# iden3/snarkjs

Hardware: NVIDIA H100
Metric: groth16_proofs_per_sec (higher is better)
Workload: dtype u32x8 (256-bit modular integers, 32-bit limbs)

## Files before the change

### snarkjs_b200/csrc/msm.cuh

```cuda
#pragma once
#include <cuda_runtime.h>
#include "ec.cuh"
#include "msm_geom.h"

namespace sb {

static constexpr int MSM_SEG = 32;
static constexpr int MSM_ACC_THREADS = 128;
static constexpr int MSM_RED_CHUNK = 16;
static constexpr uint32_t MSM_INVALID_KEY = 0xffffffffu;
static constexpr int MSM_COUNTS_SEG = 8;

extern int g_msm_force_c;

__host__ inline MsmGeom msm_choose(uint64_t n, uint32_t scalar_bytes, int fr_bits, bool precomp) {
    int eff = (int)(8 * scalar_bytes) < fr_bits ? (int)(8 * scalar_bytes) : fr_bits;
    int best_c = 3; double best = 1e300;
    for (int c = 3; c <= 22; c++) {
        int weff = (eff + 1 + c - 1) / c, top = eff + 1 - (weff - 1) * c;
        if (weff > 1 && top < c - 5) continue;
        double buckets = (precomp ? 1.0 : (double)weff) * (double)(1u << (c - 1));
        double cost = (double)weff * (double)n * 10.0 + buckets * 60.0;
        if (cost < best) { best = cost; best_c = c; }
    }
    if (g_msm_force_c) best_c = g_msm_force_c;
    MsmGeom g; g.c = best_c; g.W = (int)((8 * scalar_bytes + 1 + best_c - 1) / best_c); g.B = 1u << (best_c - 1);
    return g;
}
__host__ inline MsmGeom msm_geometry_precomp(uint64_t n_set, uint32_t scalar_bytes, int fr_bits = 254) {
    int l2 = 0; while ((1ull << (l2 + 1)) <= n_set) l2++;
    int cmax = l2; if (cmax > 22) cmax = 22; if (cmax < 8) cmax = 8;
    int c = 8;
    for (int cc = cmax; cc >= 8; cc--) {
        int weff = (fr_bits + 1 + cc - 1) / cc, top = fr_bits + 1 - (weff - 1) * cc;
        if (weff > 1 && top < cc - 5) continue;
        c = cc; break;
    }
    if (g_msm_force_c) c = g_msm_force_c;
    MsmGeom g; g.c = c; g.W = (int)((8 * scalar_bytes + 1 + c - 1) / c); g.B = 1u << (c - 1);
    g.precomp = 1; g.stride = n_set; g.first = 0;
    return g;
}
__host__ inline MsmGeom msm_geometry(uint64_t n, uint32_t scalar_bytes, int fr_bits = 254) {
    return msm_choose(n, scalar_bytes, fr_bits, false);
}

template <class F> __device__ __forceinline__ void load_affine(const Affine<F>* __restrict__ bases, uint32_t idx, F& x, F& y) {
    constexpr int NV = sizeof(F) / 16;
    const uint4* p = reinterpret_cast<const uint4*>(bases + idx);
    uint4* dx = reinterpret_cast<uint4*>(&x);
    uint4* dy = reinterpret_cast<uint4*>(&y);
#pragma unroll
    for (int k = 0; k < NV; k++) dx[k] = __ldg(p + k);
#pragma unroll
    for (int k = 0; k < NV; k++) dy[k] = __ldg(p + NV + k);
}
template <class T> __device__ __forceinline__ void store_vec(T* dst, const T& v) {
    constexpr int NV = sizeof(T) / 16;
    const uint4* s = reinterpret_cast<const uint4*>(&v);
    uint4* d = reinterpret_cast<uint4*>(dst);
#pragma unroll
    for (int k = 0; k < NV; k++) d[k] = s[k];
}
template <class T> __device__ __forceinline__ T load_vec(const T* src) {
    constexpr int NV = sizeof(T) / 16;
    T v; const uint4* s = reinterpret_cast<const uint4*>(src);
    uint4* d = reinterpret_cast<uint4*>(&v);
#pragma unroll
    for (int k = 0; k < NV; k++) d[k] = s[k];
    return v;
}

template <class P> __device__ __forceinline__ Fp<P> PairInvF(const Fp<P>& a) { return Fp<P>::inv_binary(a); }
template <class P> __device__ __forceinline__ Fp2<P> PairInvF(const Fp2<P>& a) { return Fp2<P>::inv(a); }

template <class F, int MINB>
__global__ void __launch_bounds__(MSM_ACC_THREADS, MINB)
k_accumulate(const Affine<F>* __restrict__ bases, const uint32_t* __restrict__ keys, const uint32_t* __restrict__ vals,
             const uint64_t* __restrict__ counts, XYZZ<F>* __restrict__ buckets,
             XYZZ<F>* __restrict__ heads, uint32_t* __restrict__ head_keys) {
    const uint64_t M = counts[0];
    const uint32_t seg = (uint32_t)counts[MSM_COUNTS_SEG];
    uint64_t t = blockIdx.x * (uint64_t)blockDim.x + threadIdx.x;
    uint64_t lo = t * seg;
    if (lo >= M) return;
    uint64_t hi = lo + seg < M ? lo + seg : M;
    const F one = F::one();
    XYZZ<F> acc = XYZZ<F>::inf();
    uint32_t cur = keys[lo];
    bool first = true;
    for (uint64_t e = lo; e < hi; e++) {
        uint32_t k = keys[e], v = vals ? vals[e] : (uint32_t)e;
        if (k != cur) {
            if (first) { store_vec(heads + t, acc); head_keys[t] = cur; first = false; }
            else store_vec(buckets + cur, acc);
            acc = XYZZ<F>::inf(); cur = k;
        }
        F px, py;
        load_affine<F>(bases, v & 0x7fffffffu, px, py);
        if (!(px.is_zero() & py.is_zero())) {
            py = F::cneg(py, (v >> 31) != 0);
            acc.add_affine(px, py, one);
        }
    }
    if (first) { store_vec(heads + t, acc); head_keys[t] = cur; }
    else store_vec(buckets + cur, acc);
}

static constexpr int MSM_SHORT_RUN = 8;
template <class F, int MINB>
__global__ void __launch_bounds__(MSM_ACC_THREADS, MINB)
k_fold_short(const XYZZ<F>* __restrict__ heads, const uint32_t* __restrict__ keys_in, uint32_t* __restrict__ keys_out,
             const uint64_t* __restrict__ counts, XYZZ<F>* __restrict__ buckets) {
    const uint64_t M = counts[1];
    uint64_t t = blockIdx.x * (uint64_t)blockDim.x + threadIdx.x;
    if (t >= M) return;
    const uint32_t k = keys_in[t];
    uint64_t start = t; int back = 0;
    while (start > 0 && back < MSM_SHORT_RUN && keys_in[start - 1] == k) { start--; back++; }
    bool is_short = back < MSM_SHORT_RUN;
    uint64_t len = 0;
    if (is_short) {
        len = 1;
        while (start + len < M && len <= (uint64_t)MSM_SHORT_RUN && keys_in[start + len] == k) len++;
        is_short = len <= (uint64_t)MSM_SHORT_RUN;
    }
    keys_out[t] = is_short ? MSM_INVALID_KEY : k;
    if (!is_short || start != t) return;
    XYZZ<F> acc = load_vec(buckets + k);
    for (uint64_t e = 0; e < len; e++) { XYZZ<F> p = load_vec(heads + t + e); acc.add_i(p); }
    store_vec(buckets + k, acc);
}

template <class F>
__global__ void __launch_bounds__(MSM_ACC_THREADS)
k_fold(const XYZZ<F>* __restrict__ in, const uint32_t* __restrict__ in_keys, const uint64_t* __restrict__ counts, int level,
       XYZZ<F>* __restrict__ buckets, XYZZ<F>* __restrict__ heads, uint32_t* __restrict__ head_keys) {
    const uint64_t M = counts[level];
    const bool last = M <= MSM_SEG;
    uint64_t t = blockIdx.x * (uint64_t)blockDim.x + threadIdx.x;
    uint64_t lo = t * MSM_SEG;
    if (lo >= M) return;
    uint64_t hi = lo + MSM_SEG < M ? lo + MSM_SEG : M;
    XYZZ<F> acc = XYZZ<F>::inf();
    uint32_t cur = in_keys[lo];
    bool first = !last;
    auto flush = [&]() __attribute__((always_inline)) {
        if (first) { store_vec(heads + t, acc); head_keys[t] = cur; first = false; }
        else if (cur != MSM_INVALID_KEY) { XYZZ<F> b = load_vec(buckets + cur); b.add_i(acc); store_vec(buckets + cur, b); }
    };
    for (uint64_t e = lo; e < hi; e++) {
        uint32_t k = in_keys[e];
        if (k != cur) { flush(); acc = XYZZ<F>::inf(); cur = k; }
        if (k != MSM_INVALID_KEY) { XYZZ<F> p = load_vec(in + e); acc.add_i(p); }
    }
    flush();
}

template <class F>
__global__ void __launch_bounds__(128)
k_reduce(const XYZZ<F>* __restrict__ buckets, MsmGeom g, XYZZ<F>* __restrict__ partials, uint32_t ctas_per_window) {
    extern __shared__ uint4 smem_raw[];
    XYZZ<F>* sm = reinterpret_cast<XYZZ<F>*>(smem_raw);
    const uint32_t w = blockIdx.x / ctas_per_window, cta = blockIdx.x % ctas_per_window;
    const uint32_t L = g.B < (uint32_t)MSM_RED_CHUNK ? g.B : MSM_RED_CHUNK;
    const uint32_t chunks = g.B / L;
    const uint32_t j = cta * blockDim.x + threadIdx.x;
    XYZZ<F> part = XYZZ<F>::inf();
    if (j < chunks) {
        const XYZZ<F>* bk = buckets + (uint64_t)w * g.B + (uint64_t)j * L;
        XYZZ<F> run = XYZZ<F>::inf(), sum = XYZZ<F>::inf();
        for (int b = (int)L - 1; b >= 0; b--) {
            XYZZ<F> p = load_vec(bk + b);
            run.add_i(p);
            sum.add_i(run);
        }
        uint32_t k = j * L;
        if (k) {
            int top = 31 - __clz(k);
            part = run;
            for (int bit = top - 1; bit >= 0; bit--) {
                part = XYZZ<F>::dbl(part);
                if ((k >> bit) & 1) part.add_i(run);
            }
        }
        part.add_i(sum);
    }
    store_vec(sm + threadIdx.x, part);
    __syncthreads();
    for (uint32_t s = blockDim.x >> 1; s > 0; s >>= 1) {
        if (threadIdx.x < s) {
            XYZZ<F> a = load_vec(sm + threadIdx.x), b = load_vec(sm + threadIdx.x + s);
            a.add_i(b);
            store_vec(sm + threadIdx.x, a);
        }
        __syncthreads();
    }
    if (threadIdx.x == 0) store_vec(partials + (uint64_t)w * ctas_per_window + cta, load_vec(sm));
}

template <class F>
__global__ void __launch_bounds__(32)
k_window_sum(const XYZZ<F>* __restrict__ partials, uint32_t per_window, XYZZ<F>* __restrict__ out) {
    extern __shared__ uint4 smem_raw[];
    XYZZ<F>* sm = reinterpret_cast<XYZZ<F>*>(smem_raw);
    XYZZ<F> acc = XYZZ<F>::inf();
    for (uint32_t i = threadIdx.x; i < per_window; i += 32) { XYZZ<F> p = load_vec(partials + (uint64_t)blockIdx.x * per_window + i); acc.add_i(p); }
    store_vec(sm + threadIdx.x, acc);
    __syncwarp();
    for (uint32_t s = 16; s > 0; s >>= 1) {
        if (threadIdx.x < s) { XYZZ<F> a = load_vec(sm + threadIdx.x), b = load_vec(sm + threadIdx.x + s); a.add_i(b); store_vec(sm + threadIdx.x, a); }
        __syncwarp();
    }
    if (threadIdx.x == 0) store_vec(out + blockIdx.x, load_vec(sm));
}


struct AxisJob { const void* in; void* out; uint64_t total; uint32_t S; uint32_t log_inner; };

template <class F, int MINB>
__global__ void __launch_bounds__(128, MINB)
k_axis_sum(AxisJob j0, AxisJob j1) {
    const AxisJob j = blockIdx.y ? j1 : j0;
    const uint64_t gid = blockIdx.x * (uint64_t)blockDim.x + threadIdx.x;
    if (gid >= j.total) return;
    const uint64_t o = gid >> j.log_inner, i = gid & ((1ull << j.log_inner) - 1);
    const XYZZ<F>* p = (const XYZZ<F>*)j.in + ((o * j.S) << j.log_inner) + i;
    XYZZ<F> acc = load_vec(p);
#pragma unroll 1
    for (uint32_t s = 1; s < j.S; s++) { XYZZ<F> v = load_vec(p + ((uint64_t)s << j.log_inner)); acc.add_i(v); }
    store_vec((XYZZ<F>*)j.out + gid, acc);
}

template <class F> __device__ __forceinline__ XYZZ<F> shfl_down_pt(const XYZZ<F>& v, int d) {
    constexpr int NW32 = sizeof(XYZZ<F>) / 4;
    union U { XYZZ<F> p; uint32_t w[NW32]; __device__ U() {} };
    U a, r; a.p = v;
#pragma unroll
    for (int k = 0; k < NW32; k++) r.w[k] = __shfl_down_sync(0xffffffffu, a.w[k], d);
    return r.p;
}
template <class F> __device__ __forceinline__ void warp_weighted_sum(XYZZ<F> v, XYZZ<F>& T, XYZZ<F>& W) {
    const int lane = threadIdx.x & 31;
#pragma unroll 1
    for (int d = 1; d < 32; d <<= 1) { XYZZ<F> o = shfl_down_pt<F>(v, d); if (lane + d < 32) v.add_i(o); }
    T = v;
    XYZZ<F> x = lane ? v : XYZZ<F>::inf();
#pragma unroll 1
    for (int d = 16; d >= 1; d >>= 1) { XYZZ<F> o = shfl_down_pt<F>(x, d); if (lane < d) x.add_i(o); }
    W = x;
}
template <class F> __device__ __forceinline__ XYZZ<F> warp_sum(XYZZ<F> x) {
    const int lane = threadIdx.x & 31;
#pragma unroll 1
    for (int d = 16; d >= 1; d >>= 1) { XYZZ<F> o = shfl_down_pt<F>(x, d); if (lane < d) x.add_i(o); }
    return x;
}

template <class F>
__global__ void __launch_bounds__(128)
k_ws_chunks(const XYZZ<F>* __restrict__ vecR, uint32_t lenR, const XYZZ<F>* __restrict__ vecC, uint32_t lenC, uint32_t NW, XYZZ<F>* __restrict__ tw) {
    const uint32_t nR = (lenR + 31) / 32, nC = (lenC + 31) / 32, per = nR + nC;
    const uint32_t wid = blockIdx.x * (blockDim.x >> 5) + (threadIdx.x >> 5), lane = threadIdx.x & 31;
    if (wid >= NW * per) return;
    const uint32_t w = wid / per, jj = wid % per;
    const bool isR = jj < nR;
    const uint32_t j = isR ? jj : jj - nR, len = isR ? lenR : lenC, idx = j * 32 + lane;
    const XYZZ<F>* vec = (isR ? vecR : vecC) + (uint64_t)w * len;
    XYZZ<F> v = XYZZ<F>::inf();
    if (idx < len) v = load_vec(vec + idx);
    XYZZ<F> T, W;
    warp_weighted_sum<F>(v, T, W);
    if (lane == 0) { store_vec(tw + 2 * (uint64_t)wid, T); store_vec(tw + 2 * (uint64_t)wid + 1, W); }
}

template <class F>
__global__ void __launch_bounds__(128)
k_ws_final(const XYZZ<F>* __restrict__ tw, uint32_t nR, uint32_t nC, XYZZ<F>* __restrict__ out) {
    const uint32_t warp = threadIdx.x >> 5, lane = threadIdx.x & 31, per = nR + nC;
    const XYZZ<F>* base = tw + 2 * (uint64_t)blockIdx.x * per;
    const bool r_side = warp < 2;
    const uint32_t cnt = r_side ? nR : nC, off = r_side ? 0 : nR;
    XYZZ<F> v = XYZZ<F>::inf();
    if (lane < cnt) v = load_vec(base + 2 * (uint64_t)(off + lane) + (warp & 1));
    XYZZ<F>* o = out + 5 * (uint64_t)blockIdx.x;
    if ((warp & 1) == 0) {
        XYZZ<F> tot, res;
        warp_weighted_sum<F>(v, tot, res);
        if (lane == 0) { store_vec(o + (r_side ? 0 : 2), res); if (!r_side) store_vec(o + 4, tot); }
    } else {
        XYZZ<F> res = warp_sum<F>(v);
        if (lane == 0) store_vec(o + (r_side ? 1 : 3), res);
    }
}

template <class F>
__global__ void __launch_bounds__(128)
k_axis_tree(AxisJob j0, AxisJob j1) {
    const AxisJob j = blockIdx.y ? j1 : j0;
    const uint64_t wid = blockIdx.x * (uint64_t)(blockDim.x >> 5) + (threadIdx.x >> 5);
    const uint32_t lane = threadIdx.x & 31;
    if (wid >= j.total) return;
    const uint64_t o = wid >> j.log_inner, i = wid & ((1ull << j.log_inner) - 1);
    const XYZZ<F>* p = (const XYZZ<F>*)j.in + ((o * j.S) << j.log_inner) + i;
    XYZZ<F> acc = XYZZ<F>::inf();
#pragma unroll 1
    for (uint32_t s = lane; s < j.S; s += 32) { XYZZ<F> v = load_vec(p + ((uint64_t)s << j.log_inner)); acc.add_i(v); }
    acc = warp_sum<F>(acc);
    if (lane == 0) store_vec((XYZZ<F>*)j.out + wid, acc);
}

extern int g_msm_force_reduce;

static constexpr int WS_COL_BITS = 10;
struct WsPlan {
    bool ok = false;
    int m = 0, er = 0, ec = 0;
    int levels = 0; int br[8] = {0}, bc[8] = {0};
    uint32_t lenR = 0, lenC = 0, nR = 0, nC = 0;
    size_t rowA = 0, rowB = 0, colA = 0, colB = 0, tw = 0;
    size_t elems() const { return rowA + rowB + colA + colB + tw + 8; }
};
__host__ inline WsPlan ws_plan(const MsmGeom& g) {
    WsPlan p; const int cbits = g.c - 1; const size_t NW = g.windows();
    if (cbits > 2 * WS_COL_BITS || cbits < 0) return p;
    p.ok = true;
    if (cbits > WS_COL_BITS) { p.m = WS_COL_BITS; p.er = p.m; p.ec = cbits - p.m; p.lenR = 1u << p.ec; p.lenC = 1u << p.m; }
    else { p.lenR = 0; p.lenC = g.B; }
    int rr = p.er, rc = p.ec;
    for (int l = 0; l < 2 && (rr > 0 || rc > 0); l++) {
        p.levels++;
        p.br[l] = l == 0 ? (rr < 3 ? rr : 3) : rr; p.bc[l] = l == 0 ? (rc < 3 ? rc : 3) : rc; rr -= p.br[l]; rc -= p.bc[l];
        const size_t orow = p.br[l] ? (NW * g.B) >> (p.er - rr) : 0, ocol = p.bc[l] ? (NW * g.B) >> (p.ec - rc) : 0;
        if (l & 1) { p.rowB = orow; p.colB = ocol; } else { p.rowA = orow; p.colA = ocol; }
    }
    p.nR = (p.lenR + 31) / 32; p.nC = (p.lenC + 31) / 32;
    p.tw = 2 * NW * (p.nR + p.nC);
    return p;
}
__host__ inline uint32_t msm_wsum_parts(const MsmGeom& g) { return (ws_plan(g).ok && !g_msm_force_reduce) ? 5u : 1u; }
__host__ inline size_t msm_reduce_scratch_elems(const MsmGeom& g) {
    const uint32_t NW = g.windows();
    const uint32_t L = g.B < (uint32_t)MSM_RED_CHUNK ? g.B : MSM_RED_CHUNK;
    const uint32_t ctas_per_window = (g.B / L + 127) / 128;
    const size_t legacy = (size_t)2 * NW * ctas_per_window;
    const WsPlan p = ws_plan(g);
    return (p.ok && p.elems() > legacy) ? p.elems() : legacy;
}

template <class F>
__global__ void __launch_bounds__(128) k_precompute(const Affine<F>* __restrict__ bases, uint64_t n, int c, int W, Affine<F>* __restrict__ table) {
    uint64_t i = blockIdx.x * (uint64_t)blockDim.x + threadIdx.x;
    if (i >= n) return;
    Affine<F> a = load_vec(bases + i);
    store_vec(table + i, a);
    if (a.is_inf()) {
        for (int w = 1; w < W; w++) store_vec(table + (uint64_t)w * n + i, a);
        return;
    }
    XYZZ<F> p; p.x = a.x; p.y = a.y; p.zz = F::one(); p.zzz = F::one();
    for (int w = 1; w < W; w++) {
        for (int j = 0; j < c; j++) p = XYZZ<F>::dbl(p);
        Affine<F> o;
        if (p.is_inf()) { o.x = F::zero(); o.y = F::zero(); }
        else { F t = PairInvF(F::mul(p.zz, p.zzz)); o.x = F::mul(p.x, F::mul(t, p.zzz)); o.y = F::mul(p.y, F::mul(t, p.zz)); p.x = o.x; p.y = o.y; p.zz = F::one(); p.zzz = F::one(); }
        store_vec(table + (uint64_t)w * n + i, o);
    }
}

__host__ __device__ inline uint64_t splitmix64(uint64_t x) {
    x += 0x9E3779B97F4A7C15ull; x = (x ^ (x >> 30)) * 0xBF58476D1CE4E5B9ull; x = (x ^ (x >> 27)) * 0x94D049BB133111EBull; return x ^ (x >> 31);
}
static constexpr uint64_t GEN_CHUNK = 4096;
template <class F>
__global__ void __launch_bounds__(128) k_gen_points(Affine<F> g, uint64_t seed, uint64_t n, Affine<F>* __restrict__ out) {
    uint64_t i = blockIdx.x * (uint64_t)blockDim.x + threadIdx.x;
    if (i >= n) return;
    const uint64_t c = i / GEN_CHUNK, j = i % GEN_CHUNK;
    const uint64_t k0 = (seed ^ 0x9E3779B97F4A7C15ull) + c * 0xD1B54A32D192ED03ull, kd = seed * 2654435761ull + 12345ull;
    uint64_t lo = j * kd, hi = __umul64hi(j, kd);
    lo += k0; hi += lo < k0 ? 1 : 0;
    const F one = F::one();
    XYZZ<F> r = XYZZ<F>::inf();
    for (int bit = 79; bit >= 0; bit--) {
        r = XYZZ<F>::dbl(r);
        const uint64_t wd = bit >= 64 ? hi : lo;
        if ((wd >> (bit & 63)) & 1) r.add_affine(g.x, g.y, one);
    }
    Affine<F> a;
    if (r.is_inf()) { a.x = F::zero(); a.y = F::zero(); }
    else { F t = PairInvF(F::mul(r.zz, r.zzz)); a.x = F::mul(r.x, F::mul(t, r.zzz)); a.y = F::mul(r.y, F::mul(t, r.zz)); }
    store_vec(out + i, a);
}

struct MsmScratch {
    void* p = nullptr; size_t cap = 0;
    void* get(size_t bytes) {
        if (bytes > cap) { if (p) cudaFree(p); p = nullptr; cap = 0; if (cudaMalloc(&p, bytes) != cudaSuccess) return nullptr; cap = bytes; }
        return p;
    }
    void release() { if (p) cudaFree(p); p = nullptr; cap = 0; }
};


struct MsmLaunchStats {
    int launches = 0;
    cudaEvent_t* ev = nullptr; int nev = 0; int used = 0; int tag[128] = {0}; int cur_tag = 0;
};
enum { PROF_ACC_G1 = 1, PROF_ACC_G2 = 2, PROF_SORT = 3, PROF_FOLD = 4, PROF_REDUCE = 5, PROF_QAP = 6, PROF_NTT = 7, PROF_JOIN = 8,
       PROF_FOLD_G2 = 9, PROF_REDUCE_G2 = 10 };
struct ProfScope {
    MsmLaunchStats* s; cudaStream_t st; int idx = -1;
    ProfScope(MsmLaunchStats* s_, int tag, cudaStream_t st_) : s(s_), st(st_) {
        if (s && s->ev && s->used + 2 <= s->nev && s->used / 2 < 128) { idx = s->used; s->used += 2; s->tag[idx / 2] = tag; cudaEventRecord(s->ev[idx], st); }
    }
    void end() { if (idx >= 0) { cudaEventRecord(s->ev[idx + 1], st); idx = -1; } }
    void end(cudaStream_t other) { st = other; end(); }
};

struct MsmSorted {
    const uint32_t* keys = nullptr; const uint32_t* vals = nullptr; const uint64_t* counts = nullptr;
    uint64_t n = 0, total = 0; MsmGeom g{};
    uint32_t seg_lo = MSM_SEG;
};

int msm_sort_entries(const uint8_t* d_scalars, uint32_t sbytes, uint64_t n, MsmGeom g, MsmScratch& scratch,
                     cudaStream_t stream, MsmSorted* out, MsmLaunchStats* stats);

template <class F>
int msm_buckets(const Affine<F>* d_bases, const MsmSorted& s, MsmScratch& scratch, cudaStream_t stream,
                XYZZ<F>* d_wsum, MsmLaunchStats* stats, cudaStream_t tail_stream = nullptr, cudaEvent_t ev_acc = nullptr) {
    const MsmGeom g = s.g;
    const uint32_t NW = g.windows();
    const uint64_t nbuckets = (uint64_t)NW * g.B;
    const uint64_t heads0 = (s.total + s.seg_lo - 1) / s.seg_lo;
    const uint64_t heads1 = (heads0 + MSM_SEG - 1) / MSM_SEG;
    const uint32_t L = g.B < (uint32_t)MSM_RED_CHUNK ? g.B : MSM_RED_CHUNK;
    const uint32_t chunks = g.B / L;
    const uint32_t red_threads = 128;
    const uint32_t ctas_per_window = (chunks + red_threads - 1) / red_threads;
    auto al = [](size_t x) { return (x + 255) & ~(size_t)255; };
    size_t o_buckets = 0;
    size_t o_headsA = o_buckets + al(nbuckets * sizeof(XYZZ<F>)), o_hkA = o_headsA + al(heads0 * sizeof(XYZZ<F>));
    size_t o_headsB = o_hkA + al(heads0 * 4), o_hkB = o_headsB + al(heads1 * sizeof(XYZZ<F>));
    size_t o_hkM = o_hkB + al(heads1 * 4);
    size_t o_part = o_hkM + al(heads0 * 4);
    size_t bytes = o_part + al(msm_reduce_scratch_elems(g) * sizeof(XYZZ<F>));
    uint8_t* base = (uint8_t*)scratch.get(bytes);
    if (!base) return (int)cudaErrorMemoryAllocation;
    XYZZ<F>* buckets = (XYZZ<F>*)(base + o_buckets);
    XYZZ<F>* headsA = (XYZZ<F>*)(base + o_headsA); uint32_t* hkA = (uint32_t*)(base + o_hkA);
    XYZZ<F>* headsB = (XYZZ<F>*)(base + o_headsB); uint32_t* hkB = (uint32_t*)(base + o_hkB);
    XYZZ<F>* partials = (XYZZ<F>*)(base + o_part);
    uint32_t* hkM = (uint32_t*)(base + o_hkM);
    int launches = 0;
    const bool g2 = stats && stats->cur_tag == PROF_ACC_G2;
    constexpr int TAIL_MINB = sizeof(F) > 32 ? 2 : 4;
    cudaMemsetAsync(buckets, 0, nbuckets * sizeof(XYZZ<F>), stream);
    if (heads0) {
        ProfScope prof(stats, stats ? stats->cur_tag : 0, stream);
        {
            const unsigned grid = (unsigned)((heads0 + MSM_ACC_THREADS - 1) / MSM_ACC_THREADS);
            constexpr int MINB = sizeof(F) > 32 ? 2 : 4;
            k_accumulate<F, MINB><<<grid, MSM_ACC_THREADS, 0, stream>>>(d_bases, s.keys, s.vals, s.counts, buckets, headsA, hkA);
            launches++;
        }
        prof.end();
        if (tail_stream && tail_stream != stream && ev_acc) {
            cudaEventRecord(ev_acc, stream); cudaStreamWaitEvent(tail_stream, ev_acc, 0); stream = tail_stream;
        }
        ProfScope pfold(stats, g2 ? PROF_FOLD_G2 : PROF_FOLD, stream);
        k_fold_short<F, TAIL_MINB><<<(unsigned)((heads0 + MSM_ACC_THREADS - 1) / MSM_ACC_THREADS), MSM_ACC_THREADS, 0, stream>>>(
            headsA, hkA, hkM, s.counts, buckets); launches++;
        uint64_t m = heads0; int level = 1;
        XYZZ<F>* hin = headsA; uint32_t* kin = hkM; XYZZ<F>* hout = headsB; uint32_t* kout = hkB;
        while (true) {
            uint64_t threads = (m + MSM_SEG - 1) / MSM_SEG;
            k_fold<F><<<(unsigned)((threads + MSM_ACC_THREADS - 1) / MSM_ACC_THREADS), MSM_ACC_THREADS, 0, stream>>>(
                hin, kin, s.counts, level, buckets, hout, kout); launches++;
            if (m <= (uint64_t)MSM_SEG) break;
            m = threads; level++;
            XYZZ<F>* th = hin; hin = hout; hout = th; uint32_t* tk = kin; kin = kout; kout = tk;
            if (level >= 8) return (int)cudaErrorUnknown;
        }
        pfold.end();
    }
    if (!heads0 && tail_stream && tail_stream != stream && ev_acc) { cudaEventRecord(ev_acc, stream); cudaStreamWaitEvent(tail_stream, ev_acc, 0); stream = tail_stream; }
    ProfScope pred(stats, g2 ? PROF_REDUCE_G2 : PROF_REDUCE, stream);
    const WsPlan wp = ws_plan(g);
    if (msm_wsum_parts(g) == 5) {
        XYZZ<F>* rowb[2] = {partials, partials + wp.rowA};
        XYZZ<F>* colb[2] = {partials + wp.rowA + wp.rowB, partials + wp.rowA + wp.rowB + wp.colA};
        XYZZ<F>* tw = partials + wp.rowA + wp.rowB + wp.colA + wp.colB;
        const XYZZ<F>* rin = buckets; const XYZZ<F>* cin = buckets;
        int rr = wp.er, rc = wp.ec;
        for (int l = 0; l < wp.levels; l++) {
            AxisJob jr{nullptr, nullptr, 0, 1, 0}, jc{nullptr, nullptr, 0, 1, 0};
            if (wp.br[l]) { rr -= wp.br[l]; jr = AxisJob{rin, rowb[l & 1], (uint64_t)nbuckets >> (wp.er - rr), 1u << wp.br[l], (uint32_t)rr}; rin = rowb[l & 1]; }
            if (wp.bc[l]) { rc -= wp.bc[l]; jc = AxisJob{cin, colb[l & 1], (uint64_t)nbuckets >> (wp.ec - rc), 1u << wp.bc[l], (uint32_t)wp.m}; cin = colb[l & 1]; }
            const uint64_t mx = jr.total > jc.total ? jr.total : jc.total;
            if (l == 0) k_axis_sum<F, TAIL_MINB><<<dim3((unsigned)((mx + 127) / 128), 2), 128, 0, stream>>>(jr, jc);
            else k_axis_tree<F><<<dim3((unsigned)((mx + 3) / 4), 2), 128, 0, stream>>>(jr, jc);
            launches++;
        }
        const uint32_t per = wp.nR + wp.nC;
        k_ws_chunks<F><<<(NW * per + 3) / 4, 128, 0, stream>>>(wp.lenR ? rin : nullptr, wp.lenR, cin, wp.lenC, NW, tw); launches++;
        k_ws_final<F><<<NW, 128, 0, stream>>>(tw, wp.nR, wp.nC, d_wsum); launches++;
    } else {
        k_reduce<F><<<NW * ctas_per_window, red_threads, red_threads * sizeof(XYZZ<F>), stream>>>(buckets, g, partials, ctas_per_window); launches++;
        k_window_sum<F><<<NW, 32, 32 * sizeof(XYZZ<F>), stream>>>(partials, ctas_per_window, d_wsum); launches++;
    }
    pred.end();
    if (stats) stats->launches += launches;
    return (int)cudaGetLastError();
}

}
```

Baseline: 42.46.

## Use warp ballots for run detection in fold_short and skip fold when no long runs

Rewrites k_fold_short so each warp finds run boundaries with shuffle and ballot instead of every thread scanning neighbouring keys in global memory. Only lanes 0 and 31 scan beyond the warp edges. It also sets a device flag whenever a long run exists, and k_fold returns at once when the flag is clear, so the multi-level fold does no work in the common case. The flag costs one extra memset word, and k_fold blocks are still launched to read it. A profiling script for the tail kernels is added.

```diff
diff --git a/profiles/prof_tail_kernels.py b/profiles/prof_tail_kernels.py
--- /dev/null
+++ b/profiles/prof_tail_kernels.py
@@ -0,0 +1,137 @@
+import json, os, re, subprocess, sys
+sys.path.insert(0, os.path.dirname(os.path.dirname(os.path.abspath(__file__))))
+import numpy as np
+import torch
+import snarkjs_b200
+from snarkjs_b200 import groth16, synth
+from snarkjs_b200.curve import _ptr
+
+L = int(os.environ.get("LOGN", "20"))
+WARM = int(os.environ.get("WARM", "3"))
+MULEQ = {"g1": 14.5, "g2": 39.3}
+KERNELS = ("k_fold_short", "k_fold", "k_axis_sum", "k_axis_tree", "k_ws_chunks", "k_ws_final")
+MSM_SEG, ACC_THREADS, WS_COL_BITS = 32, 128, 10
+
+
+def gpu():
+    o = subprocess.run(["nvidia-smi", "--query-gpu=name,power.limit", "--format=csv,noheader", "-i", "0"], capture_output=True, text=True)
+    return o.stdout.strip()
+
+
+def precomp_c(n_set, fr_bits=254):
+    l2 = n_set.bit_length() - 1
+    cmax = min(max(l2, 8), 22)
+    for cc in range(cmax, 7, -1):
+        weff = (fr_bits + 1 + cc - 1) // cc
+        if weff > 1 and fr_bits + 1 - (weff - 1) * cc < cc - 5:
+            continue
+        return cc
+    return 8
+
+
+def heads(M, n_buckets, total, sms):
+    T = MSM_SEG
+    while T < 256 and total // n_buckets > 2 * T:
+        T <<= 1
+    seg_lo = 16 if T == MSM_SEG else T // 2
+    wave = sms * 4 * ACC_THREADS
+    k = (M + wave * T - 1) // (wave * T)
+    seg = (M + k * wave - 1) // (k * wave) if 0 < k <= 3 else T
+    seg = min(max(seg, seg_lo), T)
+    return (M + seg - 1) // seg
+
+
+def reduce_adds(c):
+    cbits = c - 1
+    B = 1 << cbits
+    if cbits > WS_COL_BITS:
+        m, er, ec = WS_COL_BITS, WS_COL_BITS, cbits - WS_COL_BITS
+        lenR, lenC = 1 << ec, 1 << m
+    else:
+        m, er, ec, lenR, lenC = 0, 0, cbits, 0, B
+    out = {"k_axis_sum": 0, "k_axis_tree": 0}
+    rr, rc = er, ec
+    for lvl in range(2):
+        if rr <= 0 and rc <= 0:
+            break
+        br = min(rr, 3) if lvl == 0 else rr
+        bc = min(rc, 3) if lvl == 0 else rc
+        rr, rc = rr - br, rc - bc
+        name = "k_axis_sum" if lvl == 0 else "k_axis_tree"
+        if br:
+            out[name] += (B >> (er - rr)) * ((1 << br) - 1)
+        if bc:
+            out[name] += (B >> (ec - rc)) * ((1 << bc) - 1)
+    chunks = (lenR + 31) // 32 + (lenC + 31) // 32
+    out["k_ws_chunks"] = chunks * (129 + 31)
+    out["k_ws_final"] = 2 * (129 + 31) + 2 * 31
+    return out
+
+
+def main():
+    c = snarkjs_b200.getCurveFromName("bn128")
+    lib, h = c.lib, c.handle
+    zkey = synth.synth_groth16_zkey(c, L, seed=1)
+    pk = groth16.ProvingKey(zkey, curve=c)
+    w = synth.chain_witness(c.r, L)
+    n_vars = w.size // 32
+    r = (5 * (1 << 256) % c.r).to_bytes(32, "little")
+    s = (7 * (1 << 256) % c.r).to_bytes(32, "little")
+    proof = np.empty(256, np.uint8)
+    torch.cuda.init()
+    sms = torch.cuda.get_device_properties(0).multi_processor_count
+    lib.sb_set_tuning(2, 1)
+    for _ in range(WARM):
+        c.check(lib.sb_groth16_prove(h, pk.handle, _ptr(w), n_vars, r, s, _ptr(proof)))
+    torch.cuda.synchronize()
+    from torch.profiler import profile, ProfilerActivity
+    with profile(activities=[ProfilerActivity.CUDA]) as prof:
+        c.check(lib.sb_groth16_prove(h, pk.handle, _ptr(w), n_vars, r, s, _ptr(proof)))
+        torch.cuda.synchronize()
+    Mw, g1_entries = lib.sb_last_stat(h, 5), lib.sb_last_stat(h, 4)
+    Mh = g1_entries - 3 * Mw
+    lib.sb_set_tuning(2, 0)
+    peak = lib.sb_calibrate(h, 1)
+    pk.release()
+    c.terminate()
+
+    times = {}
+    for ev in prof.key_averages():
+        m = re.search(r"\b(k_fold_short|k_fold|k_axis_sum|k_axis_tree|k_ws_chunks|k_ws_final)\b", ev.key)
+        if not m:
+            continue
+        grp = "g2" if "Fp2" in ev.key else "g1"
+        t = times.setdefault((grp, m.group(1)), [0.0, 0])
+        t[0] += ev.device_time_total / 1e3
+        t[1] += ev.count
+    cw, ch = precomp_c(n_vars), precomp_c(1 << L)
+    Mw, Mh = int(Mw), int(Mh)
+    msms = {"g1": [(Mw, cw, n_vars)] * 3 + [(Mh, ch, 1 << L)], "g2": [(Mw, cw, n_vars)]}
+    res = {"gpu": gpu(), "log_n": L, "sm_count": sms, "calibrate_modmul_per_s": peak, "entries": {"witness": Mw, "h": Mh},
+           "window_bits": {"witness": cw, "h": ch}, "kernels": {}}
+    tail_ms = 0.0
+    for grp in ("g1", "g2"):
+        for k in KERNELS:
+            if (grp, k) not in times:
+                continue
+            ms, launches = times[(grp, k)]
+            adds = 0
+            for M, cc, npts in msms[grp]:
+                if k == "k_fold_short":
+                    adds += heads(M, 1 << (cc - 1), npts * ((8 * 32 + cc) // cc), sms)
+                elif k != "k_fold":
+                    adds += reduce_adds(cc)[k]
+            rate = adds * MULEQ[grp] / (ms * 1e-3) if ms > 0 else 0.0
+            res["kernels"][f"{grp}.{k}"] = {"ms": ms, "launches": launches, "additions": adds,
+                                            "modmul_per_s": rate, "frac_of_calibrated": rate / peak if peak > 0 else None}
+            tail_ms += ms
+    res["tail_ms"] = tail_ms
+    print(json.dumps(res, indent=1))
+    if os.environ.get("OUT"):
+        os.makedirs(os.environ["OUT"], exist_ok=True)
+        with open(os.path.join(os.environ["OUT"], "prof_tail_kernels.json"), "w") as f:
+            json.dump(res, f, indent=1)
+
+
+if __name__ == "__main__":
+    main()
diff --git a/snarkjs_b200/csrc/msm.cuh b/snarkjs_b200/csrc/msm.cuh
--- a/snarkjs_b200/csrc/msm.cuh
+++ b/snarkjs_b200/csrc/msm.cuh
@@ -111,31 +111,40 @@
 template <class F, int MINB>
 __global__ void __launch_bounds__(MSM_ACC_THREADS, MINB)
 k_fold_short(const XYZZ<F>* __restrict__ heads, const uint32_t* __restrict__ keys_in, uint32_t* __restrict__ keys_out,
-             const uint64_t* __restrict__ counts, XYZZ<F>* __restrict__ buckets) {
+             const uint64_t* __restrict__ counts, XYZZ<F>* __restrict__ buckets, uint32_t* __restrict__ long_runs) {
     const uint64_t M = counts[1];
-    uint64_t t = blockIdx.x * (uint64_t)blockDim.x + threadIdx.x;
-    if (t >= M) return;
-    const uint32_t k = keys_in[t];
-    uint64_t start = t; int back = 0;
-    while (start > 0 && back < MSM_SHORT_RUN && keys_in[start - 1] == k) { start--; back++; }
-    bool is_short = back < MSM_SHORT_RUN;
-    uint64_t len = 0;
-    if (is_short) {
-        len = 1;
-        while (start + len < M && len <= (uint64_t)MSM_SHORT_RUN && keys_in[start + len] == k) len++;
-        is_short = len <= (uint64_t)MSM_SHORT_RUN;
-    }
+    const uint64_t t = blockIdx.x * (uint64_t)blockDim.x + threadIdx.x, t0 = t & ~31ull;
+    if (t0 >= M) return;
+    const int lane = threadIdx.x & 31;
+    const bool valid = t < M;
+    const uint32_t k = valid ? keys_in[t] : MSM_INVALID_KEY;
+    uint32_t prev = __shfl_up_sync(0xffffffffu, k, 1);
+    if (lane == 0) prev = t0 ? keys_in[t0 - 1] : ~k;
+    const uint32_t starts = __ballot_sync(0xffffffffu, !valid || prev != k);
+    const uint32_t upto = starts & (0xffffffffu >> (31 - lane));
+    const uint32_t after = starts & ~(0xffffffffu >> (31 - lane));
+    const int s = upto ? 31 - __clz(upto) : -1;
+    const int e = after ? __ffs(after) - 1 : 32;
+    int back = 0, fwd = 0;
+    if (lane == 0 && !(starts & 1u)) { back = 1; while (back < MSM_SHORT_RUN && t0 > (uint64_t)back && keys_in[t0 - 1 - back] == k) back++; }
+    if (lane == 31 && valid) { while (fwd <= MSM_SHORT_RUN && t + 1 + fwd < M && keys_in[t + 1 + fwd] == k) fwd++; }
+    back = __shfl_sync(0xffffffffu, back, 0); fwd = __shfl_sync(0xffffffffu, fwd, 31);
+    if (!valid) return;
+    const int len = (s < 0 ? back : 0) + e - (s < 0 ? 0 : s) + (e == 32 ? fwd : 0);
+    const bool is_short = len <= MSM_SHORT_RUN;
     keys_out[t] = is_short ? MSM_INVALID_KEY : k;
-    if (!is_short || start != t) return;
+    if (s != lane) return;
+    if (!is_short) { *long_runs = 1u; return; }
     XYZZ<F> acc = load_vec(buckets + k);
-    for (uint64_t e = 0; e < len; e++) { XYZZ<F> p = load_vec(heads + t + e); acc.add_i(p); }
+    for (int i = 0; i < len; i++) { XYZZ<F> p = load_vec(heads + t + i); acc.add_i(p); }
     store_vec(buckets + k, acc);
 }
 
 template <class F>
 __global__ void __launch_bounds__(MSM_ACC_THREADS)
 k_fold(const XYZZ<F>* __restrict__ in, const uint32_t* __restrict__ in_keys, const uint64_t* __restrict__ counts, int level,
-       XYZZ<F>* __restrict__ buckets, XYZZ<F>* __restrict__ heads, uint32_t* __restrict__ head_keys) {
+       XYZZ<F>* __restrict__ buckets, XYZZ<F>* __restrict__ heads, uint32_t* __restrict__ head_keys, const uint32_t* __restrict__ long_runs) {
+    if (!*long_runs) return;
     const uint64_t M = counts[level];
     const bool last = M <= MSM_SEG;
     uint64_t t = blockIdx.x * (uint64_t)blockDim.x + threadIdx.x;
@@ -440,8 +449,8 @@
     const uint32_t red_threads = 128;
     const uint32_t ctas_per_window = (chunks + red_threads - 1) / red_threads;
     auto al = [](size_t x) { return (x + 255) & ~(size_t)255; };
-    size_t o_buckets = 0;
-    size_t o_headsA = o_buckets + al(nbuckets * sizeof(XYZZ<F>)), o_hkA = o_headsA + al(heads0 * sizeof(XYZZ<F>));
+    size_t o_buckets = 0, o_long = o_buckets + al(nbuckets * sizeof(XYZZ<F>));
+    size_t o_headsA = o_long + al(4), o_hkA = o_headsA + al(heads0 * sizeof(XYZZ<F>));
     size_t o_headsB = o_hkA + al(heads0 * 4), o_hkB = o_headsB + al(heads1 * sizeof(XYZZ<F>));
     size_t o_hkM = o_hkB + al(heads1 * 4);
     size_t o_part = o_hkM + al(heads0 * 4);
@@ -453,10 +462,11 @@
     XYZZ<F>* headsB = (XYZZ<F>*)(base + o_headsB); uint32_t* hkB = (uint32_t*)(base + o_hkB);
     XYZZ<F>* partials = (XYZZ<F>*)(base + o_part);
     uint32_t* hkM = (uint32_t*)(base + o_hkM);
+    uint32_t* long_runs = (uint32_t*)(base + o_long);
     int launches = 0;
     const bool g2 = stats && stats->cur_tag == PROF_ACC_G2;
     constexpr int TAIL_MINB = sizeof(F) > 32 ? 2 : 4;
-    cudaMemsetAsync(buckets, 0, nbuckets * sizeof(XYZZ<F>), stream);
+    cudaMemsetAsync(buckets, 0, o_long + 4, stream);
     if (heads0) {
         ProfScope prof(stats, stats ? stats->cur_tag : 0, stream);
         {
@@ -471,13 +481,13 @@
         }
         ProfScope pfold(stats, g2 ? PROF_FOLD_G2 : PROF_FOLD, stream);
         k_fold_short<F, TAIL_MINB><<<(unsigned)((heads0 + MSM_ACC_THREADS - 1) / MSM_ACC_THREADS), MSM_ACC_THREADS, 0, stream>>>(
-            headsA, hkA, hkM, s.counts, buckets); launches++;
+            headsA, hkA, hkM, s.counts, buckets, long_runs); launches++;
         uint64_t m = heads0; int level = 1;
         XYZZ<F>* hin = headsA; uint32_t* kin = hkM; XYZZ<F>* hout = headsB; uint32_t* kout = hkB;
         while (true) {
             uint64_t threads = (m + MSM_SEG - 1) / MSM_SEG;
             k_fold<F><<<(unsigned)((threads + MSM_ACC_THREADS - 1) / MSM_ACC_THREADS), MSM_ACC_THREADS, 0, stream>>>(
-                hin, kin, s.counts, level, buckets, hout, kout); launches++;
+                hin, kin, s.counts, level, buckets, hout, kout, long_runs); launches++;
             if (m <= (uint64_t)MSM_SEG) break;
             m = threads; level++;
             XYZZ<F>* th = hin; hin = hout; hout = th; uint32_t* tk = kin; kin = kout; kout = tk;
```

Result: no change. 42.53, median of 6 (+0.2%).
